# can-lehmann/exprgrad

Measured on AMD Instinct MI355X. Metric: GFLOP/s matmul 4096^3 f32 (1 GPU), higher is better.
Workload: dtype f32

## Files before the change

### exprgrad_amd/csrc/kernels/gemm_split_bf16.hip

```cpp
#include <algorithm>
#include <cfloat>

#include "gemm_fused.hpp"
#include "../eg_internal.hpp"
#include "../switches.hpp"

namespace {

typedef __bf16 bf16x8 __attribute__((ext_vector_type(8)));
typedef float f32x4 __attribute__((ext_vector_type(4)));


struct SplitOperand {
  const float* src;
  long ld;
  long R;
  int kc;
  __bf16* dst;
};

__device__ __forceinline__ void unit_coords(const SplitOperand& o, long K, long u, long& r, long& chunk) {
  const long cpr = K / 8, t = u >> 6;
  const int l = (int)(u & 63);
  if (o.kc) {
    const long per = cpr / 4;
    r = (t / per) * 16 + (l >> 2);
    chunk = (t % per) * 4 + (l & 3);
  } else {
    const long per = cpr / 2;
    r = (t / per) * 32 + (l >> 1);
    chunk = (t % per) * 2 + (l & 1);
  }
}

__device__ __forceinline__ void load_unit(const SplitOperand& o, long r, long chunk, float (&x)[8]) {
  if (o.kc) {
    const f32x4* p = reinterpret_cast<const f32x4*>(o.src + r * o.ld + chunk * 8);
    const f32x4 v0 = __builtin_nontemporal_load(p), v1 = __builtin_nontemporal_load(p + 1);
#pragma unroll
    for (int j = 0; j < 4; ++j) {
      x[j] = v0[j];
      x[4 + j] = v1[j];
    }
  } else {
    const float* p = o.src + chunk * 8 * o.ld + r;
#pragma unroll
    for (int j = 0; j < 8; ++j) x[j] = __builtin_nontemporal_load(p + j * o.ld);
  }
}

__device__ __forceinline__ void split_unit(const SplitOperand& o, long K, long r, long chunk, const float (&x)[8], bool& bad) {
  bf16x8 h0, h1, h2;
#pragma unroll
  for (int j = 0; j < 8; ++j) {
    const float v = x[j];
    const __bf16 b0 = (__bf16)v;
    const float r1 = v - (float)b0;
    const __bf16 b1 = (__bf16)r1;
    const float f1 = (float)b1;
    const float r2 = r1 - f1;
    const __bf16 b2 = (__bf16)r2;
    const float f2 = (float)b2;
    bad |= !(r2 == f2);
    bad |= v != 0.f && __builtin_fabsf(v) < FLT_MIN;
    bad |= (f1 != 0.f && __builtin_fabsf(f1) < FLT_MIN) || (f2 != 0.f && __builtin_fabsf(f2) < FLT_MIN);
    h0[j] = b0;
    h1[j] = b1;
    h2[j] = b2;
  }
  const long plane = o.R * K;
  bf16x8* d = reinterpret_cast<bf16x8*>(o.dst + ((chunk >> 1) * o.R + r) * 16 + (chunk & 1) * 8);
  const long ps = plane / 8;
  d[0] = h0;
  d[ps] = h1;
  d[2 * ps] = h2;
}

constexpr int SPLIT_NT = 256;
constexpr int SPLIT_U = 2;

__global__ __launch_bounds__(SPLIT_NT) void split_planes_kernel(SplitOperand a, SplitOperand b, long K, long units_a, long units,
                                                              unsigned* flag, unsigned epoch) {
  constexpr long STEP = (long)SPLIT_NT * SPLIT_U;
  const long per = ((units + gridDim.x - 1) / gridDim.x + STEP - 1) / STEP * STEP;
  const long lo = (long)blockIdx.x * per, hi = lo + per < units ? lo + per : units;
  bool bad = false;
  for (long base = lo; base < hi; base += STEP) {
    float x[SPLIT_U][8];
    long r[SPLIT_U], c[SPLIT_U];
#pragma unroll
    for (int i = 0; i < SPLIT_U; ++i) {
      const long u = base + i * SPLIT_NT + threadIdx.x;
      if (u >= hi) continue;
      const bool in_a = u < units_a;
      unit_coords(in_a ? a : b, K, in_a ? u : u - units_a, r[i], c[i]);
      load_unit(in_a ? a : b, r[i], c[i], x[i]);
    }
#pragma unroll
    for (int i = 0; i < SPLIT_U; ++i) {
      const long u = base + i * SPLIT_NT + threadIdx.x;
      if (u >= hi) continue;
      split_unit(u < units_a ? a : b, K, r[i], c[i], x[i], bad);
    }
  }
  if (__builtin_expect(bad, 0)) *(volatile unsigned*)flag = epoch;
}


constexpr int BM = 256, BN = 256, WM = 128, WN = 64, NT = 512;
constexpr int STAGES = 3;
constexpr int PLANE_BYTES = BM * 16 * 2;
constexpr int STAGE_BYTES = 6 * PLANE_BYTES;
constexpr int LOADS = STAGE_BYTES / (NT * 16);

struct SplitGemmArgs {
  const __bf16* pa;
  const __bf16* pb;
  float* C;
  const float* bias;
  long M, N, K, ldc;
  int tiles_m, tiles_n;
  int accumulate;
  int skew;
  const unsigned* flag;
  unsigned epoch;
};

__device__ __forceinline__ int xcd_remap(int bid, int nwg) {
  constexpr int NXCD = 8;
  const int q = nwg / NXCD, r = nwg % NXCD;
  const int xcd = bid % NXCD, local = bid / NXCD;
  return (xcd < r ? xcd * (q + 1) : r * (q + 1) + (xcd - r) * q) + local;
}
__device__ __forceinline__ void tile_origin(int wgid, int tiles_m, int tiles_n, long& m_blk, long& n_blk) {
  constexpr int GROUP = 8;
  const int per_group = GROUP * tiles_n;
  const int first_m = (wgid / per_group) * GROUP;
  const int gsize = min(tiles_m - first_m, GROUP);
  const int in_group = wgid % per_group;
  m_blk = (long)(first_m + in_group % gsize) * BM;
  n_blk = (long)(in_group / gsize) * BN;
}

__device__ __forceinline__ const void* uniform_ptr(const void* p) {
  const unsigned long v = reinterpret_cast<unsigned long>(p);
  const unsigned lo = __builtin_amdgcn_readfirstlane((unsigned)v), hi = __builtin_amdgcn_readfirstlane((unsigned)(v >> 32));
  return reinterpret_cast<const void*>(((unsigned long)hi << 32) | lo);
}

constexpr int ROLE_LOAD_OWN = 1, ROLE_LOAD_PARTNER = 2, ROLE_READ_TOP = 4, ROLE_READ_AHEAD = 8;
constexpr int PARTNER = 4;

#ifdef EG_SPLIT_GEMM_STAMPS
constexpr int STAMP_BLOCKS = 1024;
__device__ unsigned long long g_split_stamps[STAMP_BLOCKS][8][4];
#define EG_STAMP(t)                                                                  \
  do {                                                                               \
    __builtin_amdgcn_sched_barrier(0);                                               \
    asm volatile("s_memtime %0\n\ts_waitcnt lgkmcnt(0)" : "=s"(t)::"memory"); \
    __builtin_amdgcn_sched_barrier(0);                                               \
  } while (0)
#else
#define EG_STAMP(t) \
  do {              \
  } while (0)
#endif

__global__ __launch_bounds__(NT) void split_gemm_kernel(SplitGemmArgs a) {
  if (*(volatile const unsigned*)a.flag == a.epoch) return;
  __shared__ __attribute__((aligned(16))) unsigned char lds[STAGES * STAGE_BYTES];

  const int tid = threadIdx.x, lane = tid & 63, wave = __builtin_amdgcn_readfirstlane(tid >> 6);
  const int wr = wave >> 2, wc = wave & 3;
  long m_blk, n_blk;
  tile_origin(xcd_remap(blockIdx.x, gridDim.x), a.tiles_m, a.tiles_n, m_blk, n_blk);

  const __amdgpu_buffer_rsrc_t ra = __builtin_amdgcn_make_buffer_rsrc(
      const_cast<void*>(uniform_ptr(a.pa + m_blk * 16)), (short)0, -1, 0x00020000);
  const __amdgpu_buffer_rsrc_t rb = __builtin_amdgcn_make_buffer_rsrc(
      const_cast<void*>(uniform_ptr(a.pb + n_blk * 16)), (short)0, -1, 0x00020000);
  const unsigned a_plane = (unsigned)(a.M * a.K * 2), b_plane = (unsigned)(a.N * a.K * 2);
  const unsigned a_ktile = (unsigned)(a.M * 32), b_ktile = (unsigned)(a.N * 32);
  const unsigned voff = (unsigned)lane * 16;

  auto pieces = [&](int kt, int s, int w) {
    unsigned char* st = lds + s * STAGE_BYTES + w * 1024;
    const unsigned at = (unsigned)kt * a_ktile + (unsigned)w * 1024, bt = (unsigned)kt * b_ktile + (unsigned)w * 1024;
#pragma unroll
    for (int i = 0; i < LOADS; ++i) {
      __attribute__((address_space(3))) void* dst = (__attribute__((address_space(3))) void*)(st + i * PLANE_BYTES);
      if (i < 3)
        __builtin_amdgcn_raw_ptr_buffer_load_lds(ra, dst, 16, voff, (unsigned)i * a_plane + at, 0, 0);
      else
        __builtin_amdgcn_raw_ptr_buffer_load_lds(rb, dst, 16, voff, (unsigned)(i - 3) * b_plane + bt, 0, 0);
    }
  };
  auto issue = [&](int kt, int s, int r) {
    if (r & ROLE_LOAD_OWN) pieces(kt, s, wave);
    if (r & ROLE_LOAD_PARTNER) pieces(kt, s, wave ^ PARTNER);
  };

  f32x4 acc[8][4];
#pragma unroll
  for (int i = 0; i < 8; ++i)
#pragma unroll
    for (int j = 0; j < 4; ++j)
#pragma unroll
      for (int r = 0; r < 4; ++r) acc[i][j][r] = 0.f;

  const int sel = lane >> 5;
  const int a_row = (wr * WM + (lane & 15)) * 32 + ((lane >> 4) & 1) * 16;
  const int b_row = 3 * PLANE_BYTES + (wc * WN + (lane & 15)) * 32 + ((lane >> 4) & 1) * 16;
  const int a01_off = a_row + sel * PLANE_BYTES, a02_off = a_row + 2 * sel * PLANE_BYTES;
  const int b21_off = b_row + (2 - sel) * PLANE_BYTES, b10_off = b_row + (1 - sel) * PLANE_BYTES, b00_off = b_row;

  bf16x8 fb21[4], fb10[4], fb00[4], fa01, fa02;
  auto read_head = [&](const unsigned char* st) {
#pragma unroll
    for (int j = 0; j < 4; ++j) {
      fb21[j] = *reinterpret_cast<const bf16x8*>(st + b21_off + j * 512);
      fb10[j] = *reinterpret_cast<const bf16x8*>(st + b10_off + j * 512);
      fb00[j] = *reinterpret_cast<const bf16x8*>(st + b00_off + j * 512);
    }
    fa01 = *reinterpret_cast<const bf16x8*>(st + a01_off);
    fa02 = *reinterpret_cast<const bf16x8*>(st + a02_off);
  };
#pragma unroll
  for (int j = 0; j < 4; ++j) fb21[j] = fb10[j] = fb00[j] = bf16x8{};
  fa01 = fa02 = bf16x8{};

  const int skew = a.skew;
  const int role = !skew ? ROLE_LOAD_OWN | ROLE_READ_TOP
                         : (wave & PARTNER) ? ROLE_LOAD_OWN | ROLE_LOAD_PARTNER | ROLE_READ_TOP : ROLE_READ_AHEAD;
  const int KT = (int)(a.K / 16);
  issue(0, 0, role);
  if (KT > 1) issue(1, 1, role);
  if (skew) {
    if (KT > 1) asm volatile("s_waitcnt vmcnt(12)" ::: "memory");
    else asm volatile("s_waitcnt vmcnt(0)" ::: "memory");
    __builtin_amdgcn_s_barrier();
    asm volatile("" ::: "memory");
    if (role & ROLE_READ_AHEAD) read_head(lds);
  }
#ifdef EG_SPLIT_GEMM_STAMPS
  unsigned long long t0 = 0, t1 = 0, t2 = 0, front = 0, body = 0, back = 0;
#endif
  int s = 0;
  for (int kt = 0; kt < KT; ++kt) {
    if (!skew && kt + 1 < KT) asm volatile("s_waitcnt vmcnt(6)" ::: "memory");
    else asm volatile("s_waitcnt vmcnt(0)" ::: "memory");
    __builtin_amdgcn_s_barrier();
    asm volatile("" ::: "memory");
#ifdef EG_SPLIT_GEMM_STAMPS
    EG_STAMP(t0);
    if (kt) back += t0 - t2;
#endif
    int r = role;
    asm volatile("" : "+s"(r));
    if (kt + 2 < KT) issue(kt + 2, s == 0 ? 2 : s - 1, r);
    const unsigned char* st = lds + s * STAGE_BYTES;
    if (r & ROLE_READ_TOP) read_head(st);
    EG_STAMP(t1);
    bf16x8 c01 = fa01, c02 = fa02;
#pragma unroll
    for (int i = 0; i < 8; ++i) {
      bf16x8 n01 = c01, n02 = c02;
      __builtin_amdgcn_sched_barrier(0);
      if (i + 1 < 8) {
        n01 = *reinterpret_cast<const bf16x8*>(st + a01_off + (i + 1) * 512);
        n02 = *reinterpret_cast<const bf16x8*>(st + a02_off + (i + 1) * 512);
      }
      __builtin_amdgcn_sched_barrier(0);
#pragma unroll
      for (int j = 0; j < 4; ++j) acc[i][j] = __builtin_amdgcn_mfma_f32_16x16x32_bf16(c01, fb21[j], acc[i][j], 0, 0, 0);
#pragma unroll
      for (int j = 0; j < 4; ++j) acc[i][j] = __builtin_amdgcn_mfma_f32_16x16x32_bf16(c01, fb10[j], acc[i][j], 0, 0, 0);
#pragma unroll
      for (int j = 0; j < 4; ++j) acc[i][j] = __builtin_amdgcn_mfma_f32_16x16x32_bf16(c02, fb00[j], acc[i][j], 0, 0, 0);
      c01 = n01;
      c02 = n02;
    }
    EG_STAMP(t2);
#ifdef EG_SPLIT_GEMM_STAMPS
    front += t1 - t0;
    body += t2 - t1;
#endif
    s = s == STAGES - 1 ? 0 : s + 1;
    if ((r & ROLE_READ_AHEAD) && kt + 1 < KT) read_head(lds + s * STAGE_BYTES);
  }
#ifdef EG_SPLIT_GEMM_STAMPS
  if (lane == 0 && blockIdx.x < STAMP_BLOCKS) {
    unsigned long long* o = g_split_stamps[blockIdx.x][wave];
    o[0] = front;
    o[1] = body;
    o[2] = back;
    o[3] = (unsigned long long)KT;
  }
#endif

  __syncthreads();
  float* park = reinterpret_cast<float*>(lds) + wave * 64 * WN;
  const int prow = lane >> 4, pc4 = (lane & 15) * 4;
  const long col = n_blk + wc * WN + pc4;
  f32x4 b4 = {0.f, 0.f, 0.f, 0.f};
  if (a.bias) b4 = *reinterpret_cast<const f32x4*>(a.bias + col);
#pragma unroll
  for (int h = 0; h < 2; ++h) {
#pragma unroll
    for (int i = 0; i < 4; ++i)
#pragma unroll
      for (int j = 0; j < 4; ++j)
#pragma unroll
        for (int r = 0; r < 4; ++r) park[(i * 16 + 4 * prow + r) * WN + j * 16 + (lane & 15)] = acc[4 * h + i][j][r];
    asm volatile("s_waitcnt lgkmcnt(0)" ::: "memory");
#pragma unroll
    for (int q = 0; q < 16; ++q) {
      const int row = 4 * q + prow;
      f32x4 v = *reinterpret_cast<const f32x4*>(park + row * WN + pc4);
      f32x4* c = reinterpret_cast<f32x4*>(a.C + (m_blk + wr * WM + h * 64 + row) * a.ldc + col);
      if (a.accumulate) v = *c + v;
      if (a.bias) v = v + b4;
      *c = v;
    }
    asm volatile("s_waitcnt lgkmcnt(0)" ::: "memory");
  }
}

inline bool aligned16(const void* p) { return (reinterpret_cast<uintptr_t>(p) & 15) == 0; }

constexpr size_t kPlaneCap = 1ull << 30;

}

namespace eg {
namespace gemm {

int sgemm_split(eg_ctx* ctx, int trans_a, int trans_b, long M, long N, long K, const float* A, long lda, const float* B, long ldb,
                float* C, long ldc, int accumulate, const float* bias) {
  if (!ctx || !A || !B || !C || M <= 0 || N <= 0 || K <= 0) return EG_ERR_UNSUPPORTED;
  if (lda < (trans_a ? M : K) || ldb < (trans_b ? K : N) || ldc < N) return EG_ERR_UNSUPPORTED;
  if (eg::sw::on("EG_NO_SPLIT_GEMM")) return EG_ERR_UNSUPPORTED;
  if (M % BM != 0 || N % BN != 0 || K % 32 != 0 || K < 2048) return EG_ERR_UNSUPPORTED;
  if ((M / BM) * (N / BN) < ctx->compute_units) return EG_ERR_UNSUPPORTED;
  const size_t plane_bytes = 6 * (size_t)(M + N) * (size_t)K;
  if (plane_bytes > kPlaneCap || 6 * (size_t)std::max(M, N) * (size_t)K >= (1ull << 31)) return EG_ERR_UNSUPPORTED;
  if (!aligned16(A) || !aligned16(B) || (!trans_a && lda % 4 != 0) || (trans_b && ldb % 4 != 0)) return EG_ERR_UNSUPPORTED;
  if (!aligned16(C) || ldc % 4 != 0 || (bias && !aligned16(bias))) return EG_ERR_UNSUPPORTED;
  if (!exact_single_launch(ctx, trans_a, trans_b, M, N, K, A, lda, B, ldb, C, ldc, bias)) return EG_ERR_UNSUPPORTED;

  int rc = eg::set_device(ctx);
  if (rc) return rc;
  if (!ctx->split_flag) {
    EG_HIP_CHECK(hipMalloc((void**)&ctx->split_flag, sizeof(unsigned)));
    EG_HIP_CHECK(hipMemset(ctx->split_flag, 0, sizeof(unsigned)));
  }
  rc = eg::ensure_workspace(ctx, plane_bytes);
  if (rc) return rc;
  if (++ctx->split_epoch == 0) ctx->split_epoch = 1;
  const unsigned epoch = ctx->split_epoch;

  __bf16* pa = static_cast<__bf16*>(ctx->workspace);
  __bf16* pb = pa + 3 * (size_t)M * K;
  const SplitOperand oa = {A, lda, M, trans_a ? 0 : 1, pa};
  const SplitOperand ob = {B, ldb, N, trans_b ? 1 : 0, pb};
  const long units_a = M * K / 8, units = (M + N) * K / 8;
  long blocks = (units + SPLIT_NT * SPLIT_U - 1) / (SPLIT_NT * SPLIT_U);
  if (blocks > 8L * ctx->compute_units) blocks = 8L * ctx->compute_units;
  hipLaunchKernelGGL(split_planes_kernel, dim3((unsigned)blocks), dim3(SPLIT_NT), 0, ctx->stream, oa, ob, K, units_a, units,
                     ctx->split_flag, epoch);
  EG_HIP_CHECK(hipGetLastError());

  SplitGemmArgs g = {};
  g.pa = pa;
  g.pb = pb;
  g.C = C;
  g.bias = bias;
  g.M = M;
  g.N = N;
  g.K = K;
  g.ldc = ldc;
  g.tiles_m = (int)(M / BM);
  g.tiles_n = (int)(N / BN);
  g.accumulate = accumulate;
  g.skew = eg::sw::present("EG_GEMM_NO_SKEW") ? 0 : 1;
  g.flag = ctx->split_flag;
  g.epoch = epoch;
  hipLaunchKernelGGL(split_gemm_kernel, dim3((unsigned)(g.tiles_m * g.tiles_n)), dim3(NT), 0, ctx->stream, g);
  EG_HIP_CHECK(hipGetLastError());

  return sgemm_exact(ctx, trans_a, trans_b, M, N, K, A, lda, B, ldb, C, ldc, accumulate, bias, ctx->split_flag, epoch);
}

}
}

#ifdef EG_SPLIT_GEMM_STAMPS
extern "C" int eg_debug_split_stamps(unsigned long long* dst, size_t count) {
  if (count > sizeof(g_split_stamps) / sizeof(unsigned long long)) return EG_ERR_UNSUPPORTED;
  EG_HIP_CHECK(hipDeviceSynchronize());
  EG_HIP_CHECK(hipMemcpyFromSymbol(dst, HIP_SYMBOL(g_split_stamps), count * sizeof(unsigned long long)));
  return 0;
}
#endif
```

### exprgrad_amd/csrc/switches.cpp

```cpp
#include "switches.hpp"

#include <cstdio>
#include <cstring>
#include <mutex>
#include <string>
#include <unordered_map>
#include <vector>

#include "exprgrad_hip.h"

namespace {

struct Row {
  const char* name;
  const char* cls;
  const char* purpose;
};

const Row kSwitches[] = {
    {"EG_TUNING", "execution", "honour the rows of class `tuning` (measurement aids); unset: they are ignored"},
    {"EG_NO_GRAPH", "execution", "launch one by one instead of replaying captured HIP graphs"},
    {"EG_NO_DPP_BUTTERFLY", "execution", "row groups exchange lanes through the LDS crossbar in every step of a wave reduction (no DPP moves)"},
    {"EG_NO_DEFERRED_FOLD", "execution", "a row group in front of a side-lane group folds its partial rows itself, not on the side lane"},
    {"EG_NO_OVERLAP", "execution", "no side lane: bandwidth-bound launches run in front of the long contraction, not next to it"},
    {"EG_NO_ROWFUSE", "execution", "no row / sample / map / small fusion groups: one launch per kernel"},
    {"EG_NO_EPILOGUE", "execution", "elementwise consumers of a contraction stay their own launches"},
    {"EG_NO_INLINE", "execution", "no producer / consumer inlining of elementwise kernels into generated kernels"},
    {"EG_NO_ALIAS", "execution", "whole-tensor raw copies (reshape) are copied instead of sharing storage"},
    {"EG_NO_ONES_ROW", "execution", "bias gradient as its own column sum instead of the weight gradient's virtual row of ones"},
    {"EG_NO_SMALL_GEMM", "execution", "tiny contractions on the matrix tiles instead of one wave per output element"},
    {"EG_NO_NARROW_INDEX", "execution", "64-bit index arithmetic everywhere in generated kernels"},
    {"EG_NO_PREDICATE", "execution", "pre-activations stored as values, not as predicate bits"},
    {"EG_NO_ROW_PRODUCT", "execution", "the 10-wide forward product as its own launch, not in the previous layer's epilogue"},
    {"EG_NO_ROW_DIRECT", "execution", "a one-block row group writes a partial row for row_finalize instead of its totals"},
    {"EG_NO_SMALL_PAIR", "execution", "two independent tiny contractions as two launches"},
    {"EG_NO_SKINNY_GEMM", "execution", "N <= 16 products on the matrix tiles instead of the streaming skinny kernel"},
    {"EG_NO_NARROW_K", "execution", "K <= 16 products with a generated epilogue on the matrix tile instead of the streaming kernel"},
    {"EG_NO_SAMPLE_FUSE", "execution", "no sample groups (one block per sample): the launch chain of a small-batch step"},
    {"EG_OVERLAP_SIDE_FIRST", "execution", "the side lane's launches are issued in front of the long contraction they run beside (the order of rounds 2 - 5)"},
    {"EG_SAMPLE_KEEP_BARRIERS", "execution", "sample kernels keep the barrier between independent members"},
    {"EG_SAMPLE_NO_STAGE", "execution", "a sample group's members read parameters from global memory, not from a copy in LDS"},
    {"EG_SAMPLE_NO_MFMA", "execution", "convolution members of a sample group as scalar loop nests, not on the matrix cores"},
    {"EG_NO_SLAB_FOLD", "execution", "the optimizer's map group does not add up the sample kernel's slab rows itself"},
    {"EG_NO_SLAB_SUM", "execution", "k-slices folded by the two-launch column sum instead of slab_sum"},
    {"EG_NO_ROW_TAIL", "execution", "a row group's last block neither folds the partial rows nor runs the update"},
    {"EG_PIPELINE", "execution", "the batch pipeline (two half batches, streaming launches under the other half's contraction): OFF unless 1"},
    {"EG_NO_SPLIT_GEMM", "execution", "eg_sgemm runs every product on the exact f32 matrix path, never as three-way split bf16"},
    {"EG_GEMM_NO_SKEW", "execution", "every wave of a contraction block runs the k loop in phase (the round-3 loop)"},
    {"EG_GEMM_NO_BK32", "execution", "16-deep k-tiles for long whole-tile products"},
    {"EG_GEMM_NO_PAIR", "execution", "no wave-pair / eight-wave small-tile kernels"},
    {"EG_GEMM_NO_T96", "execution", "no 96 x 96 whole-round tiles"},
    {"EG_GEMM_NO_STREAMK", "execution", "64 x 64 tiles one block per tile, not persistent stream-K blocks"},
    {"EG_GEMM_NO_XROW", "execution", "1 .. 32 rows beyond whole tiles as a ragged tile row, not a ninth accumulator block"},
    {"EG_GEMM_NO_WIDE_STORE", "execution", "tiles leave as 128-byte pieces instead of through LDS as whole rows"},
    {"EG_CONV_NO_TINY", "execution", "small convolutions on the contraction route"},
    {"EG_CONV_NO_GRADF_HALO", "execution", "filter gradient as one gathered contraction"},
    {"EG_CONV_NO_WIDE_STORE", "execution", "halo convolution stores 128-byte pieces"},
    {"EG_CONV_NO_VIRTUAL_PAD", "execution", "image gradient reads a padded copy of the output gradient"},
    {"EG_CONV_NO_HALO", "execution", "3 x 3-class convolutions on the implicit-GEMM route"},
    {"EG_CONV_NO_DIRECT", "execution", "few-channel convolutions on the implicit-GEMM route"},
    {"EG_CONV_NO_BAND", "execution", "small-channel convolutions on the routes the band kernels replaced"},
    {"EG_NO_STAGED_COPY", "execution", "downloads into pageable memory as one runtime copy"},
    {"EG_FIT_NO_DIRECT", "execution", "fit copies every batch into the inputs' staging buffers"},
    {"EG_DP_REAGREE_STEPS", "data-parallel", "steps between two negotiations of the exchange schedule (default 256; 0: only the first)"},
    {"EG_DP_INIT_TIMEOUT_S", "data-parallel", "watchdog on ncclCommInitRank, seconds (default 180)"},
    {"EG_DP_RESERVE_CUS", "data-parallel", "compute units the tail range leaves to RCCL's kernel (default 8)"},
    {"EG_DP_TEST_AS_MULTI", "data-parallel", "a one-rank group takes the N > 1 code paths (one-GPU boxes)"},
    {"EG_DP_NO_SPLIT", "data-parallel", "groups start with the early / late split of the bucket forbidden (eg_dp_set_split)"},
    {"EG_HIPRTC_LIB", "compiler", "path of the libhiprtc the library opens"},
    {"EG_KERNEL_CACHE", "compiler", "directory of the on-disk code-object cache"},
    {"EG_NO_KERNEL_CACHE", "compiler", "no on-disk code-object cache"},
    {"EG_POISON", "detector", "NaN patterns in every scratch block and every slot that is overwritten, before each run"},
    {"EG_NO_PLAN_CHECK", "detector", "skip the plan invariants (host/plan_check.cpp)"},
    {"EG_DEBUG_GRAPH", "detector", "print graph captures, replays and refusals"},
    {"EG_DEBUG_OVERLAP", "detector", "print the side-lane groups of a plan"},
    {"EG_DEBUG_TILE", "detector", "print the tile model's estimate per candidate"},
    {"EG_DEBUG_SAMPLE", "detector", "print why a sample group did or did not form"},
    {"EG_DUMP_FUSED", "detector", "directory: generated translation units of fused contractions"},
    {"EG_DUMP_CODE", "detector", "directory: hiprtc code objects and the text they were built from"},
    {"EG_DUMP_BAND", "detector", "directory: generated band-convolution sources"},
    {"EG_GRADF_TRACE", "detector", "per-wave cycle stamps of the halo filter-gradient kernel"},
    {"EG_HALO_TRACE", "detector", "per-wave cycle stamps of the halo convolution kernel"},
    {"EG_GEMM_TRACE", "detector", "per-wave cycle stamps of the fused and the extra-row contraction kernels (k loop begins / ends, epilogue done)"},
    {"EG_ROW_TRACE", "detector", "the last block of a row group with a tail prints cycle stamps of its hand-off"},
    {"EG_SAMPLE_TRACE", "detector", "block 0 of a sample kernel prints cycle stamps behind every member's barrier"},
    {"EG_GEMM_FORCE_TILE", "tuning", "bm,bn: force the contraction tile"},
    {"EG_GEMM_FORCE_SPLITS", "tuning", "n: force the k-slice count"},
    {"EG_GEMM_OLD_TILE_MODEL", "tuning", "round-1 cost model for wide outputs"},
    {"EG_STREAMK_BLOCKS_PER_CU", "tuning", "persistent blocks per CU of a stream-K launch"},
    {"EG_STREAMK_MIN_RATIO", "tuning", "microseconds the balance model must promise before a 64 x 64 launch goes stream-K (default 24)"},
    {"EG_GEMM_SMALL_BK32", "tuning", "32-deep k-tiles for every 64 x 64 launch"},
    {"EG_DGEMM_TILE", "tuning", "config[,splits]: force the float64 tile"},
    {"EG_CONV_BAND_PIXELS", "tuning", "pixels per band of the band convolutions"},
    {"EG_CONV_DIRECT_BLOCKS", "tuning", "block cap of the direct filter gradient"},
    {"EG_ROW_TAIL_BLOCKS", "tuning", "blocks of a row group that carries a tail (default: 12 KB of rows per block, at least 64)"},
    {"EG_SAMPLE_STOP", "tuning", "k: a sample kernel ends behind member k (wrong numbers: the time of its first k + 1 members)"},
    {"EG_SAMPLE_FUSE_MAX_BATCH", "tuning", "largest batch that forms a sample group (default 1280)"},
    {"EG_EPILOGUE_MIN_ELEMS", "tuning", "smallest output that gets a generated epilogue (default 2^20; tests: 0)"},
    {"EG_PIPELINE_MIN_FLOPS", "tuning", "smallest contraction the batch pipeline cuts"},
    {"EG_FIT_GROUP", "tuning", "batches per captured graph launch in fit (1: every batch its own launch)"},
    {"EG_FIT_PIECE_BYTES", "tuning", "upload piece of fit"},
    {"EG_FIT_SEGMENT_BYTES", "tuning", "device-resident segment of fit"},
};
constexpr int kCount = (int)(sizeof(kSwitches) / sizeof(kSwitches[0]));

struct Cache {
  std::mutex mu;
  bool loaded = false;
  bool tuning = false;
  std::unordered_map<std::string, int> index;
  std::vector<std::string> value;
  std::vector<char> set;
  void load() {
    if (index.empty())
      for (int i = 0; i < kCount; ++i) index[kSwitches[i].name] = i;
    value.assign(kCount, std::string());
    set.assign(kCount, 0);
    const char* t = getenv("EG_TUNING");
    tuning = t && t[0] && t[0] != '0';
    for (int i = 0; i < kCount; ++i) {
      const char* e = getenv(kSwitches[i].name);
      if (!e) continue;
      if (!tuning && strcmp(kSwitches[i].cls, "tuning") == 0) continue;
      value[i] = e;
      set[i] = 1;
    }
    loaded = true;
    ++generation;
  }
  unsigned generation = 0;
};
Cache& cache() {
  static Cache c;
  return c;
}

}

namespace eg {
namespace sw {

const char* raw(const char* name) {
  Cache& c = cache();
  std::lock_guard<std::mutex> lock(c.mu);
  if (!c.loaded) c.load();
  auto it = c.index.find(name);
  if (it == c.index.end()) {
    fprintf(stderr, "[exprgrad_hip] switch %s is not in the table of csrc/switches.cpp: read as unset\n", name);
    return nullptr;
  }
  return c.set[it->second] ? c.value[it->second].c_str() : nullptr;
}

unsigned generation() {
  Cache& c = cache();
  std::lock_guard<std::mutex> lock(c.mu);
  if (!c.loaded) c.load();
  return c.generation;
}

void reload() {
  Cache& c = cache();
  std::lock_guard<std::mutex> lock(c.mu);
  c.load();
}

}
}

extern "C" {

int eg_switches_reload(void) {
  eg::sw::reload();
  return EG_OK;
}

int64_t eg_switch_table(char* buf, size_t cap) {
  std::string s;
  for (int i = 0; i < kCount; ++i) s += std::string(kSwitches[i].name) + "\t" + kSwitches[i].cls + "\t" + kSwitches[i].purpose + "\n";
  if (buf && cap > 0) {
    const size_t n = s.size() < cap - 1 ? s.size() : cap - 1;
    memcpy(buf, s.data(), n);
    buf[n] = 0;
  }
  return (int64_t)s.size();
}

}
```

Baseline: 251,100.

## Split strided operands through LDS-staged tiles with 16-byte loads

Adds a tiled split kernel for operands whose k dimension runs along the leading dimension. It loads 256-row by 16-k tiles as 16-byte vector loads, splits each value into three bf16 planes, and stages them in double-buffered LDS. It then writes them out in the plane layout the GEMM expects, with the next tile prefetched while the current one is stored. This replaces per-lane 4-byte strided loads in the split pre-pass, at the cost of LDS traffic, a barrier per tile and a fixed grid of three blocks per CU.

```diff
diff --git a/exprgrad_amd/csrc/kernels/gemm_split_bf16.hip b/exprgrad_amd/csrc/kernels/gemm_split_bf16.hip
--- a/exprgrad_amd/csrc/kernels/gemm_split_bf16.hip
+++ b/exprgrad_amd/csrc/kernels/gemm_split_bf16.hip
@@ -8,6 +8,7 @@
 namespace {
 
 typedef __bf16 bf16x8 __attribute__((ext_vector_type(8)));
+typedef __bf16 bf16x4 __attribute__((ext_vector_type(4)));
 typedef float f32x4 __attribute__((ext_vector_type(4)));
 
 
@@ -49,21 +50,25 @@
   }
 }
 
+__device__ __forceinline__ void split_elem(float v, __bf16& b0, __bf16& b1, __bf16& b2, bool& bad) {
+  b0 = (__bf16)v;
+  const float r1 = v - (float)b0;
+  b1 = (__bf16)r1;
+  const float f1 = (float)b1;
+  const float r2 = r1 - f1;
+  b2 = (__bf16)r2;
+  const float f2 = (float)b2;
+  bad |= !(r2 == f2);
+  bad |= v != 0.f && __builtin_fabsf(v) < FLT_MIN;
+  bad |= (f1 != 0.f && __builtin_fabsf(f1) < FLT_MIN) || (f2 != 0.f && __builtin_fabsf(f2) < FLT_MIN);
+}
+
 __device__ __forceinline__ void split_unit(const SplitOperand& o, long K, long r, long chunk, const float (&x)[8], bool& bad) {
   bf16x8 h0, h1, h2;
 #pragma unroll
   for (int j = 0; j < 8; ++j) {
-    const float v = x[j];
-    const __bf16 b0 = (__bf16)v;
-    const float r1 = v - (float)b0;
-    const __bf16 b1 = (__bf16)r1;
-    const float f1 = (float)b1;
-    const float r2 = r1 - f1;
-    const __bf16 b2 = (__bf16)r2;
-    const float f2 = (float)b2;
-    bad |= !(r2 == f2);
-    bad |= v != 0.f && __builtin_fabsf(v) < FLT_MIN;
-    bad |= (f1 != 0.f && __builtin_fabsf(f1) < FLT_MIN) || (f2 != 0.f && __builtin_fabsf(f2) < FLT_MIN);
+    __bf16 b0, b1, b2;
+    split_elem(x[j], b0, b1, b2, bad);
     h0[j] = b0;
     h1[j] = b1;
     h2[j] = b2;
@@ -79,28 +84,125 @@
 constexpr int SPLIT_NT = 256;
 constexpr int SPLIT_U = 2;
 
+template <int U>
+__device__ __forceinline__ void split_units(const SplitOperand& a, const SplitOperand& b, long K, long units_a, long lo, long hi,
+                                            bool& bad) {
+  constexpr long STEP = (long)SPLIT_NT * U;
+  for (long base = lo; base < hi; base += STEP) {
+    float x[U][8];
+    long r[U], c[U];
+#pragma unroll
+    for (int i = 0; i < U; ++i) {
+      const long u = base + i * SPLIT_NT + threadIdx.x;
+      if (u >= hi) continue;
+      const bool in_a = u < units_a;
+      unit_coords(in_a ? a : b, K, in_a ? u : u - units_a, r[i], c[i]);
+      load_unit(in_a ? a : b, r[i], c[i], x[i]);
+    }
+#pragma unroll
+    for (int i = 0; i < U; ++i) {
+      const long u = base + i * SPLIT_NT + threadIdx.x;
+      if (u >= hi) continue;
+      split_unit(u < units_a ? a : b, K, r[i], c[i], x[i], bad);
+    }
+  }
+}
+
 __global__ __launch_bounds__(SPLIT_NT) void split_planes_kernel(SplitOperand a, SplitOperand b, long K, long units_a, long units,
                                                               unsigned* flag, unsigned epoch) {
   constexpr long STEP = (long)SPLIT_NT * SPLIT_U;
   const long per = ((units + gridDim.x - 1) / gridDim.x + STEP - 1) / STEP * STEP;
   const long lo = (long)blockIdx.x * per, hi = lo + per < units ? lo + per : units;
   bool bad = false;
-  for (long base = lo; base < hi; base += STEP) {
-    float x[SPLIT_U][8];
-    long r[SPLIT_U], c[SPLIT_U];
-#pragma unroll
-    for (int i = 0; i < SPLIT_U; ++i) {
-      const long u = base + i * SPLIT_NT + threadIdx.x;
-      if (u >= hi) continue;
-      const bool in_a = u < units_a;
-      unit_coords(in_a ? a : b, K, in_a ? u : u - units_a, r[i], c[i]);
-      load_unit(in_a ? a : b, r[i], c[i], x[i]);
-    }
-#pragma unroll
-    for (int i = 0; i < SPLIT_U; ++i) {
-      const long u = base + i * SPLIT_NT + threadIdx.x;
-      if (u >= hi) continue;
-      split_unit(u < units_a ? a : b, K, r[i], c[i], x[i], bad);
+  split_units<SPLIT_U>(a, b, K, units_a, lo, hi, bad);
+  if (__builtin_expect(bad, 0)) *(volatile unsigned*)flag = epoch;
+}
+
+constexpr int TILE_R = 256;
+constexpr int REC_BYTES = 8 * 32 + 16;
+constexpr int IMG_PLANE = (TILE_R / 8) * REC_BYTES;
+constexpr int IMG_BYTES = 3 * IMG_PLANE;
+constexpr int TILE_BLOCKS_PER_CU = 3;
+
+__device__ __forceinline__ void load_tile(const SplitOperand& o, long kt, long rb, f32x4 (&x)[4]) {
+  const int wave = threadIdx.x >> 6, lane = threadIdx.x & 63;
+  const float* p = o.src + (kt * 16 + wave * 4) * o.ld + rb * TILE_R + lane * 4;
+#pragma unroll
+  for (int i = 0; i < 4; ++i) x[i] = __builtin_nontemporal_load(reinterpret_cast<const f32x4*>(p + i * o.ld));
+}
+
+__device__ __forceinline__ void split_tile(const f32x4 (&x)[4], unsigned char* img, bool& bad) {
+  const int wave = threadIdx.x >> 6, lane = threadIdx.x & 63;
+  unsigned char* row = img + (lane >> 1) * REC_BYTES + (lane & 1) * 128 + wave * 8;
+#pragma unroll
+  for (int c = 0; c < 4; ++c) {
+    bf16x4 h0, h1, h2;
+#pragma unroll
+    for (int i = 0; i < 4; ++i) {
+      __bf16 b0, b1, b2;
+      split_elem(x[i][c], b0, b1, b2, bad);
+      h0[i] = b0;
+      h1[i] = b1;
+      h2[i] = b2;
+    }
+    *reinterpret_cast<bf16x4*>(row + c * 32) = h0;
+    *reinterpret_cast<bf16x4*>(row + c * 32 + IMG_PLANE) = h1;
+    *reinterpret_cast<bf16x4*>(row + c * 32 + 2 * IMG_PLANE) = h2;
+  }
+}
+
+__device__ __forceinline__ int lane_unit(int lane) {
+  const int quad = (lane >> 2) & 7;
+  return ((lane >> 5) * 2 + (__builtin_popcount(quad) & 1)) * 16 + (quad >> 1) * 4 + (lane & 3);
+}
+
+__device__ __forceinline__ void store_tile(const SplitOperand& o, long K, long kt, long rb, const unsigned char* img) {
+  const int wave = threadIdx.x >> 6, lane = threadIdx.x & 63;
+  const long plane = o.R * K;
+  __bf16* d = o.dst + (kt * o.R + rb * TILE_R) * 16;
+#pragma unroll
+  for (int p = 0; p < 3; ++p)
+#pragma unroll
+    for (int i = 0; i < 2; ++i) {
+      const int u = (wave * 2 + i) * 64 + lane_unit(lane);
+      const bf16x8 v = *reinterpret_cast<const bf16x8*>(img + p * IMG_PLANE + (u >> 4) * REC_BYTES + (u & 15) * 16);
+      *reinterpret_cast<bf16x8*>(d + p * plane + u * 8) = v;
+    }
+}
+
+__global__ __launch_bounds__(SPLIT_NT) void split_tiles_kernel(SplitOperand a, SplitOperand b, long K, int tiled, unsigned* flag,
+                                                             unsigned epoch) {
+  __shared__ __attribute__((aligned(16))) unsigned char img[2][IMG_BYTES];
+  bool bad = false;
+  int s = 0;
+#pragma unroll
+  for (int which = 0; which < 2; ++which) {
+    const SplitOperand& o = which ? b : a;
+    const long n = o.R * K / (TILE_R * 16);
+    const long lo = n * blockIdx.x / gridDim.x, hi = n * (blockIdx.x + 1) / gridDim.x;
+    if (!(tiled >> which & 1)) {
+      const long units = o.R * K / 8;
+      split_units<SPLIT_U>(o, o, K, units, lo * (SPLIT_NT * 2), hi * (SPLIT_NT * 2), bad);
+      continue;
+    }
+    if (lo >= hi) continue;
+    const long tr = o.R / TILE_R;
+    long kt = lo / tr, rb = lo % tr;
+    f32x4 x[4];
+    load_tile(o, kt, rb, x);
+    for (long t = lo; t < hi; ++t) {
+      split_tile(x, img[s], bad);
+      long nkt = kt, nrb = rb + 1;
+      if (nrb == tr) {
+        nrb = 0;
+        ++nkt;
+      }
+      if (t + 1 < hi) load_tile(o, nkt, nrb, x);
+      __syncthreads();
+      store_tile(o, K, kt, rb, img[s]);
+      s ^= 1;
+      kt = nkt;
+      rb = nrb;
     }
   }
   if (__builtin_expect(bad, 0)) *(volatile unsigned*)flag = epoch;
@@ -363,11 +465,19 @@
   __bf16* pb = pa + 3 * (size_t)M * K;
   const SplitOperand oa = {A, lda, M, trans_a ? 0 : 1, pa};
   const SplitOperand ob = {B, ldb, N, trans_b ? 1 : 0, pb};
-  const long units_a = M * K / 8, units = (M + N) * K / 8;
-  long blocks = (units + SPLIT_NT * SPLIT_U - 1) / (SPLIT_NT * SPLIT_U);
-  if (blocks > 8L * ctx->compute_units) blocks = 8L * ctx->compute_units;
-  hipLaunchKernelGGL(split_planes_kernel, dim3((unsigned)blocks), dim3(SPLIT_NT), 0, ctx->stream, oa, ob, K, units_a, units,
-                     ctx->split_flag, epoch);
+  const bool scalar = eg::sw::on("EG_SPLIT_PASS_SCALAR");
+  const int tiled = (!scalar && !oa.kc && lda % 4 == 0 ? 1 : 0) | (!scalar && !ob.kc && ldb % 4 == 0 ? 2 : 0);
+  if (tiled) {
+    const long blocks = (long)TILE_BLOCKS_PER_CU * ctx->compute_units;
+    hipLaunchKernelGGL(split_tiles_kernel, dim3((unsigned)blocks), dim3(SPLIT_NT), 0, ctx->stream, oa, ob, K, tiled, ctx->split_flag,
+                       epoch);
+  } else {
+    const long units_a = M * K / 8, units = (M + N) * K / 8;
+    long blocks = (units + SPLIT_NT * SPLIT_U - 1) / (SPLIT_NT * SPLIT_U);
+    if (blocks > 8L * ctx->compute_units) blocks = 8L * ctx->compute_units;
+    hipLaunchKernelGGL(split_planes_kernel, dim3((unsigned)blocks), dim3(SPLIT_NT), 0, ctx->stream, oa, ob, K, units_a, units,
+                       ctx->split_flag, epoch);
+  }
   EG_HIP_CHECK(hipGetLastError());
 
   SplitGemmArgs g = {};
diff --git a/exprgrad_amd/csrc/switches.cpp b/exprgrad_amd/csrc/switches.cpp
--- a/exprgrad_amd/csrc/switches.cpp
+++ b/exprgrad_amd/csrc/switches.cpp
@@ -46,6 +46,7 @@
     {"EG_NO_ROW_TAIL", "execution", "a row group's last block neither folds the partial rows nor runs the update"},
     {"EG_PIPELINE", "execution", "the batch pipeline (two half batches, streaming launches under the other half's contraction): OFF unless 1"},
     {"EG_NO_SPLIT_GEMM", "execution", "eg_sgemm runs every product on the exact f32 matrix path, never as three-way split bf16"},
+    {"EG_SPLIT_PASS_SCALAR", "execution", "the split pass reads an operand whose k runs along ld as 4-byte loads per lane (units), not as 16-byte tiles through LDS"},
     {"EG_GEMM_NO_SKEW", "execution", "every wave of a contraction block runs the k loop in phase (the round-3 loop)"},
     {"EG_GEMM_NO_BK32", "execution", "16-deep k-tiles for long whole-tile products"},
     {"EG_GEMM_NO_PAIR", "execution", "no wave-pair / eight-wave small-tile kernels"},
```

Result: faster. 254,700 (median of 6 runs) (+1.4%).
